# dnbaker/bonsai

Hardware: AMD Instinct MI355X
Metric: reads/s classified (150 bp) (higher is better)
Workload: dtype u64

## Files before the change

### bonsai_amd/context.py

```python
import ctypes as C
from fractions import Fraction

import numpy as np

from . import _lib
from ._lib import BonsaiAmdError, u8p, u16p, u32p, u64p, vp


def _p(a, t):
    return a.ctypes.data_as(t)


def concat_reads(seqs):
    bs = [s.encode() if isinstance(s, str) else bytes(s) for s in seqs]
    offsets = np.zeros(len(bs) + 1, dtype=np.uint64)
    if bs:
        offsets[1:] = np.cumsum([len(b) for b in bs], dtype=np.uint64)
    bases = np.frombuffer(b"".join(bs), dtype=np.uint8).copy() if bs else np.zeros(0, dtype=np.uint8)
    return bases, offsets


def pack_reads(bases, offsets, threads=1):
    L = _lib.load()
    bases = np.ascontiguousarray(bases, dtype=np.uint8)
# ... 32 lines not shown
                                        _p(offsets, u64p), _p(words, u64p), _p(bw, u64p), _p(bm, u32p), cap, C.cast(C.byref(nb), u64p), int(threads))
        if rc == 0:
            return words, bw[:nb.value].copy(), bm[:nb.value].copy(), offsets
        if nb.value <= cap:
            raise BonsaiAmdError("bns_pack_reads_qual_ptrs: %s" % L.bns_strerror(rc).decode())
        cap = int(nb.value)


def confidence_fraction(threshold):
    if isinstance(threshold, bool):
        raise ValueError("confidence threshold must be a number in [0, 1], not %r" % (threshold,))
    if isinstance(threshold, float):
        threshold = str(threshold)
    try:
        f = Fraction(threshold)
    except (TypeError, ValueError, ZeroDivisionError):
        raise ValueError("confidence threshold must be a number in [0, 1], not %r" % (threshold,)) from None
    if not 0 <= f <= 1:
        raise ValueError("confidence threshold must lie in [0, 1], not %s" % f)
    if f.denominator >= 1 << 64:
        raise ValueError("confidence threshold %s: num and den in lowest terms must be below 2^64" % f)
    return f.numerator, f.denominator


class Context:
    def __init__(self, device=0):
        self.L = _lib.load()
        h = vp()
        rc = self.L.bns_create(device, C.byref(h))
        if rc != 0:
            raise BonsaiAmdError("bns_create(%d): %s" % (device, self.L.bns_strerror(rc).decode()))
        self.h = h
        self.k = None

    def close(self):
        if getattr(self, "h", None):
            self.L.bns_destroy(self.h)
            self.h = None

    def __del__(self):
        try:
            self.close()
        except Exception:
            pass

    def _chk(self, rc, what):
        if rc != 0:
            raise BonsaiAmdError("%s: %s (%s)" % (what, self.L.bns_strerror(rc).decode(),
                                                   self.L.bns_last_error(self.h).decode()))

    def set_encoder(self, k, gaps=None, canonicalize=True, spaced_intended=True):
        g = None
        gp = None
        if gaps is not None:
            g = np.ascontiguousarray(gaps, dtype=np.uint16)
            if g.size != k - 1:
                raise ValueError("gaps must have k-1 entries")
            gp = _p(g, u16p)
        self._chk(self.L.bns_set_encoder(self.h, k, gp, int(canonicalize), int(spaced_intended)), "bns_set_encoder")
        self.k = k

    def set_window(self, w, score=_lib.SCORE_LEX):
        self._chk(self.L.bns_set_window(self.h, w, score), "bns_set_window")

    def set_bucket_slots_log2(self, lg):
        self._chk(self.L.bns_set_bucket_slots_log2(self.h, lg), "bns_set_bucket_slots_log2")

    def set_table_buckets(self, n):
        self._chk(self.L.bns_set_table_buckets(self.h, n), "bns_set_table_buckets")

    def set_minimizer_identity(self, bits):
        self._chk(self.L.bns_set_minimizer_identity(self.h, bits), "bns_set_minimizer_identity")

    def set_table_fill(self, mode):
        self._chk(self.L.bns_set_table_fill(self.h, mode), "bns_set_table_fill")

    def table_geometry(self):
        g = (C.c_uint64 * 8)()
        self._chk(self.L.bns_table_geometry(self.h, g), "bns_table_geometry")
        return {"buckets": g[0], "m": g[1], "identity_bits": g[2], "spilled_keys": g[3], "span": g[4], "overflow_keys": g[5], "group_fill": g[6]}

    def table_warning(self):
        return self.L.bns_table_warning(self.h).decode()

    def debug_set(self, bits):
        self._chk(self.L.bns_debug_set(self.h, bits), "bns_debug_set")

    def debug_claim_waves(self, waves):
        self._chk(self.L.bns_debug_set_claim_waves(self.h, int(waves)), "bns_debug_set_claim_waves")

    def last_classify_form(self):
        w = np.zeros(18, dtype=np.uint32)
        n = self.L.bns_debug_last_classify_form(self.h, _p(w, u32p), w.size)
        if n != w.size:
            raise BonsaiAmdError("bns_debug_last_classify_form: %d words" % n)
        v = [int(x) for x in w]
        return {"kernel": tuple(v[1:9]) if v[0] else None, "overflow_kernel": tuple(v[10:14]) if v[9] else None,
                "overflow_units": v[14], "overflow_grid": v[15], "chunk": v[16], "grid": v[17]}

    def load_table(self, n_buckets, flags, keys, vals, layout=_lib.LAYOUT_MINBUCKET):
        flags = np.ascontiguousarray(flags, dtype=np.uint32)
        keys = np.ascontiguousarray(keys, dtype=np.uint64)
        vals = np.ascontiguousarray(vals, dtype=np.uint32)
        if keys.size != n_buckets or vals.size != n_buckets or flags.size != max(1, n_buckets >> 4):
            raise ValueError("khash array sizes do not match n_buckets")
        self._chk(self.L.bns_load_table(self.h, n_buckets, _p(flags, u32p), _p(keys, u64p), _p(vals, u32p), layout),
                  "bns_load_table")

    def load_table_device(self, n_buckets, d_flags, d_keys, d_vals, layout=_lib.LAYOUT_MINBUCKET, stream=None):
        self._chk(self.L.bns_load_table_device(self.h, n_buckets, d_flags, d_keys, d_vals, layout, stream),
                  "bns_load_table_device")

    def table_info(self):
        nk = C.c_uint64(); nb = C.c_uint64(); ly = C.c_int()
        self._chk(self.L.bns_table_info(self.h, C.byref(nk), C.byref(nb), C.byref(ly)), "bns_table_info")
        return {"n_keys": nk.value, "device_bytes": nb.value, "layout": ly.value}

    def table_stats(self):
        st = (C.c_uint64 * 4)()
        self._chk(self.L.bns_table_stats(self.h, st), "bns_table_stats")
        return {"n_keys": st[0], "n_overflow_keys": st[1], "main_bytes": st[2], "overflow_bytes": st[3]}

    def set_minimizer_span(self, span):
        self._chk(self.L.bns_set_minimizer_span(self.h, span), "bns_set_minimizer_span")

    def table_minimizer(self):
        m = C.c_uint32(); sp = C.c_uint64()
        self._chk(self.L.bns_table_minimizer(self.h, C.byref(m), C.byref(sp)), "bns_table_minimizer")
        return {"m": m.value, "spilled_keys": sp.value}

    def load_taxonomy(self, parent):
        parent = np.ascontiguousarray(parent, dtype=np.uint32)
        self._chk(self.L.bns_load_taxonomy(self.h, _p(parent, u32p), parent.size), "bns_load_taxonomy")
        self._n_tax = int(parent.size)

    def tally_enable(self, on=True):
        self._chk(self.L.bns_tally_enable(self.h, int(bool(on))), "bns_tally_enable")

    def tally(self, reset=False):
        n = getattr(self, "_n_tax", 0)
        direct = np.zeros(n + 1, dtype=np.uint64)
        clade = np.zeros(n + 1, dtype=np.uint64)
        self._chk(self.L.bns_tally_read(self.h, _p(direct, u64p), _p(clade, u64p), n + 1, int(bool(reset))), "bns_tally_read")
        return direct, clade

    def table_tally(self):
        n = getattr(self, "_n_tax", 0)
        direct = np.zeros(n + 1, dtype=np.uint64)
        clade = np.zeros(n + 1, dtype=np.uint64)
        self._chk(self.L.bns_table_tally(self.h, _p(direct, u64p), _p(clade, u64p), n + 1), "bns_table_tally")
        return direct, clade

    def set_confidence(self, threshold):
        num, den = confidence_fraction(threshold)
        self._chk(self.L.bns_set_confidence(self.h, num, den), "bns_set_confidence")

    def set_min_hit_groups(self, n):
        self._chk(self.L.bns_set_min_hit_groups(self.h, int(n)), "bns_set_min_hit_groups")

    def sketch_enable(self, max_taxa=65536):
        self._chk(self.L.bns_sketch_enable(self.h, int(max_taxa)), "bns_sketch_enable")

    def sketch(self, reset=False):
        s = C.c_uint32(); dropped = C.c_uint32()
        self._chk(self.L.bns_sketch_read(self.h, None, None, 0, C.byref(s), C.byref(dropped), 0), "bns_sketch_read")
        bins = np.zeros(s.value, dtype=np.uint32)
# ... 399 lines not shown
```

### bonsai_amd/csrc/bns_api.hip

```cpp
#include "../../include/bonsai_amd.h"
#include "bns_kernels.hip"
#include "bns_tally.hpp"
#include "bns_inspect.hpp"
#include "bns_confidence.hpp"
#include "bns_sketch.hpp"
#include "bns_hit_groups.hpp"
#include "bns_text_plan.hpp"

#include <dlfcn.h>
#if defined(__x86_64__)
#include <immintrin.h>
#endif
#include <rccl/rccl.h>
#include <mutex>
#include <numeric>
#include <algorithm>
#include <array>
#include <cstdio>
#include <cstdlib>
#include <cmath>
#include <cstring>
#include <string>
#include <chrono>
#include <type_traits>
#include <thread>
#include <vector>

using namespace bns;

namespace {

struct DevBuf {
    void *p = nullptr;
    size_t cap = 0;
};

struct SmallLayout {
    u32 work_counter; u32 pad0[31];
    u32 ovf_count, max_len; u32 pad1[30];
    unsigned long long load_cnt[8];
    unsigned long long runs_cursor;
    unsigned long long lines_cursor;
};
constexpr size_t SMALL_BYTES = 512;
constexpr size_t SMALL_CLASSIFY_ZERO = offsetof(SmallLayout, max_len) + sizeof(u32);
static_assert(sizeof(SmallLayout) <= SMALL_BYTES, "ctx->small is allocated with SMALL_BYTES");
static_assert(offsetof(SmallLayout, load_cnt) >= SMALL_CLASSIFY_ZERO, "classify's memset must not reach the other entry points' words");

constexpr int BNS_DBG_PEXT_OFF = 0x400;
constexpr int BNS_DBG_FORCE_RCCL = 0x800;
constexpr int BNS_DBG_INSPECT_TINY = 0x8;
constexpr int BNS_DBG_INSPECT_WHOLE = 0x80;

struct ClassifyForm {
    enum { VALID, SPACED, LAYOUT, KT, NM, SPAN, OVC, WIDE, PACKED, OVF_LAUNCHED, OVF_SPACED, OVF_LAYOUT, OVF_WIDE, OVF_PACKED, OVF_UNITS,
           OVF_GRID, CHUNK, GRID, N_WORDS };
    u32 w[N_WORDS] = {0};
};

}

struct bns_text_work;
namespace bns { struct BuildSession; }
namespace bns { struct WindowSession; }
void text_work_free(struct bns_ctx *ctx);

struct bns_ctx {
    int device = 0;
    bns_text_work *text_work = nullptr;
    bns::BuildSession *build = nullptr;
    bns::WindowSession *windows = nullptr;
    hipStream_t stream = nullptr;
    hipStream_t copy_stream = nullptr;
    hipStream_t back_stream = nullptr;
    hipEvent_t slice_ev[16] = {}, done_ev[16] = {};
    std::string err;
    int n_cu = 256;
    bool enc_set = false;
    u32 k = 0, c = 0;
    bool canon = true, spaced = false, spaced_intended = false;
    u16 pos[32] = {0};
    u32 n_runs = 0;
    u8 run_start[32] = {0}, run_len[32] = {0};
    u64 sample_mask = 0;
    u32 table_m = 0;
    u32 min_span_req = 0;
    u64 n_spilled = 0;
    bool group_fill = false;
    u32 table_len = 0, table_shift = 0, table_canon = 1;
    u32 sp_run_len = 0, sp_run_shift = 0;
    u32 pext_on = 0, pext_n1 = 0, pext_steps[2] = {0, 0}, pext_top[2] = {0xFF, 0xFF};
    u64 pext_mask[2] = {0, 0}, pext_mv[2][6] = {{0}};
    u32 win = 0;
    int score = 0;
    int layout = -1;
    u64 kh_nb = 0;
    const u32 *kflags = nullptr;
    const u64 *kkeys = nullptr;
    const u32 *kvals = nullptr;
    bool own_khash = false;
    Slot *slots = nullptr;
    u64 n_slots = 0;
    u32 n_mb = 0;
    Slot *ovf_slots = nullptr;
    u64 n_ovf_slots = 0, n_ovf_keys = 0;
    u64 n_keys = 0;
    u32 slots_log2_req = 0;
    u64 n_buckets_req = 0;
    int fill_req = -1;
    int wide_req = -1;
    bool table_wide = false;
    u32 table_span = 0;
    std::string warn;
    int dbg = 0;
    unsigned claim_waves = 0;
    ClassifyForm last_form;
    u32 table_k = 0;
    TaxNode *nodes = nullptr;
    u32 n_nodes = 0;
    u32 tax_clock = 0;
    bool tally_on = false;
    DevBuf tally_direct, tally_clade, tally_scan;
    u64 conf_num = 0, conf_den = 1;
    DevBuf conf_hits;
    u32 min_hit_groups = 0;
    u32 sketch_cap = 0;
    DevBuf sk_regs, sk_slot_of, sk_slot_bin, sk_seen, sk_state;
// ... 50 lines not shown
{
    const u64 need = (items + per_block - 1) / per_block;
    const u64 cap = (u64)ctx->n_cu * blocks_per_cu;
    return (unsigned)std::max<u64>(1, std::min(need, cap));
}

template <class F>
void dispatch_sp_layout(bool spaced, int layout, F &&f)
{
    if (spaced) {
        if (layout == 2) f(std::true_type{}, std::integral_constant<int, 2>{});
        else if (layout == 1) f(std::true_type{}, std::integral_constant<int, 1>{});
        else f(std::true_type{}, std::integral_constant<int, 0>{});
    } else {
        if (layout == 2) f(std::false_type{}, std::integral_constant<int, 2>{});
        else if (layout == 1) f(std::false_type{}, std::integral_constant<int, 1>{});
        else f(std::false_type{}, std::integral_constant<int, 0>{});
    }
}

void free_table(bns_ctx *ctx)
{
    if (ctx->own_khash) {
        if (ctx->kflags) (void)hipFree((void *)ctx->kflags);
        if (ctx->kkeys) (void)hipFree((void *)ctx->kkeys);
        if (ctx->kvals) (void)hipFree((void *)ctx->kvals);
    }
    ctx->kflags = nullptr; ctx->kkeys = nullptr; ctx->kvals = nullptr; ctx->own_khash = false; ctx->kh_nb = 0;
    if (ctx->slots) (void)hipFree(ctx->slots);
    if (ctx->ovf_slots) (void)hipFree(ctx->ovf_slots);
    ctx->ovf_slots = nullptr; ctx->n_ovf_slots = 0; ctx->n_ovf_keys = 0;
    ctx->slots = nullptr; ctx->n_slots = 0; ctx->n_mb = 0; ctx->n_keys = 0; ctx->layout = -1; ctx->table_wide = false;
}

int ready(bns_ctx *ctx, bool need_table, bool need_tax)
{
    if (!ctx) return BNS_ERR_ARG;
    if (!ctx->enc_set) return fail(ctx, BNS_ERR_STATE, "encoder not configured (bns_set_encoder)");
    if (need_table && ctx->layout < 0) return fail(ctx, BNS_ERR_STATE, "no table loaded (bns_load_table)");
    if (need_table && ctx->layout == BNS_LAYOUT_MINBUCKET && ctx->table_k != ctx->k)
        return fail(ctx, BNS_ERR_STATE, "encoder k changed after a BNS_LAYOUT_MINBUCKET table was built; reload the table");
    if (need_tax && !ctx->nodes) return fail(ctx, BNS_ERR_STATE, "no taxonomy loaded (bns_load_taxonomy)");
    return BNS_OK;
}

}

#include "bns_classify.hpp"
#include "bns_dust.hpp"
#include "bns_build.hpp"
#include "bns_fewest.hpp"
#include "bns_minimize.hpp"
#include "bns_table_load.hpp"
#include "bns_windows.hpp"
#include "bns_hashers.hpp"

extern "C" {

int bns_version(void) { return 115; }

int bns_device_pci_bus_id(int device, char *out, int cap)
{
    if (!out || cap < 16) return BNS_ERR_ARG;
    return hipDeviceGetPCIBusId(out, cap, device) == hipSuccess ? BNS_OK : BNS_ERR_HIP;
}

int bns_device_count(void)
{
    int n = 0;
    if (hipGetDeviceCount(&n) != hipSuccess) return 0;
    return n;
}

int bns_debug_set(bns_ctx *ctx, int bits) { if (!ctx) return BNS_ERR_ARG; ctx->dbg = bits; return BNS_OK; }
int bns_debug_set_claim_waves(bns_ctx *ctx, unsigned waves) { if (!ctx || (waves & 3u)) return BNS_ERR_ARG; ctx->claim_waves = waves; return BNS_OK; }
int bns_debug_last_classify_form(const bns_ctx *ctx, uint32_t *out, int n)
{
    if (!ctx || !out || n < 0) return BNS_ERR_ARG;
    const int c = std::min<int>(n, ClassifyForm::N_WORDS);
    for (int i = 0; i < c; ++i) out[i] = ctx->last_form.w[i];
    return c;
}
#ifdef BNS_WAVE_TIMES
extern "C" int bns_debug_wave_times(bns_ctx *ctx, unsigned long long *out40960)
{
    if (!ctx || !out40960) return BNS_ERR_ARG;
    if (hipDeviceSynchronize() != hipSuccess) return BNS_ERR_HIP;
    if (hipMemcpyFromSymbol(out40960, HIP_SYMBOL(bns::g_wave_times), sizeof(bns::g_wave_times)) != hipSuccess) return BNS_ERR_HIP;
    return BNS_OK;
}
#endif
#ifdef BNS_COUNT_FETCHES
__global__ void ovf_stats_kernel(const bns::Slot *ovf, unsigned long long n_slots, unsigned long long *out)
{
    const unsigned long long stride = (unsigned long long)gridDim.x * blockDim.x;
    unsigned long long occ = 0, full = 0;
    for (unsigned long long b = (unsigned long long)blockIdx.x * blockDim.x + threadIdx.x; b < n_slots / 4; b += stride) {
        unsigned c = 0;
        for (int q = 0; q < 4; ++q) c += ovf[b * 4 + q].occ ? 1u : 0u;
        occ += c; full += c == 4u;
    }
    atomicAdd(out, occ); atomicAdd(out + 1, full);
}
extern "C" int bns_debug_ovf_stats(bns_ctx *ctx, unsigned long long *out3)
{
    if (!ctx || !out3) return BNS_ERR_ARG;
    out3[0] = out3[1] = 0; out3[2] = ctx->n_ovf_slots;
    if (!ctx->ovf_slots) return BNS_OK;
    unsigned long long *d = ((SmallLayout *)ctx->small.p)->load_cnt;
    if (hipMemset(d, 0, 16) != hipSuccess) return BNS_ERR_HIP;
    hipLaunchKernelGGL(ovf_stats_kernel, dim3(1024), dim3(256), 0, 0, ctx->ovf_slots, (unsigned long long)ctx->n_ovf_slots, d);
    if (hipDeviceSynchronize() != hipSuccess) return BNS_ERR_HIP;
    if (hipMemcpy(out3, d, 16, hipMemcpyDeviceToHost) != hipSuccess) return BNS_ERR_HIP;
    return BNS_OK;
}
extern "C" int bns_debug_ovf_copy(bns_ctx *ctx, void *host, unsigned long long bytes)
{
    if (!ctx || !host || !ctx->ovf_slots) return BNS_ERR_ARG;
    const unsigned long long have = ctx->n_ovf_slots * sizeof(bns::Slot);
    if (hipMemcpy(host, ctx->ovf_slots, bytes < have ? bytes : have, hipMemcpyDeviceToHost) != hipSuccess) return BNS_ERR_HIP;
    return BNS_OK;
}
extern "C" int bns_debug_fetch_count(bns_ctx *ctx, unsigned long long *out8)
{
    if (!ctx || !out8) return BNS_ERR_ARG;
    unsigned long long z[8] = {0, 0, 0, 0, 0, 0, 0, 0};
    if (hipDeviceSynchronize() != hipSuccess) return BNS_ERR_HIP;
    if (hipMemcpyFromSymbol(out8, HIP_SYMBOL(bns::g_fetch_count), sizeof(z)) != hipSuccess) return BNS_ERR_HIP;
    if (hipMemcpyToSymbol(HIP_SYMBOL(bns::g_fetch_count), z, sizeof(z)) != hipSuccess) return BNS_ERR_HIP;
    return BNS_OK;
}
#endif

const char *bns_strerror(int code)
{
    switch (code) {
        case BNS_OK: return "ok";
        case BNS_ERR_ARG: return "bad argument";
        case BNS_ERR_HIP: return "HIP runtime error";
        case BNS_ERR_NOMEM: return "out of memory";
        case BNS_ERR_STATE: return "context not ready";
        case BNS_ERR_TAX_CYCLE: return "taxonomy contains a cycle";
        case BNS_ERR_TAX_RANGE: return "taxid out of range for the flat parent array";
        case BNS_ERR_TABLE: return "inconsistent khash table";
        case BNS_ERR_NO_DEVICE: return "no usable GPU device";
        default: return "unknown error";
    }
}

const char *bns_last_error(const bns_ctx *ctx) { return ctx ? ctx->err.c_str() : "null context"; }

int bns_create(int device, bns_ctx **out)
{
    if (!out) return BNS_ERR_ARG;
    *out = nullptr;
    int n = 0;
    if (hipGetDeviceCount(&n) != hipSuccess || n <= 0 || device < 0 || device >= n) return BNS_ERR_NO_DEVICE;
    if (hipSetDevice(device) != hipSuccess) return BNS_ERR_NO_DEVICE;
    bns_ctx *ctx = new (std::nothrow) bns_ctx();
    if (!ctx) return BNS_ERR_NOMEM;
    ctx->device = device;
    hipDeviceProp_t prop;
    if (hipGetDeviceProperties(&prop, device) == hipSuccess) ctx->n_cu = prop.multiProcessorCount > 0 ? prop.multiProcessorCount : 256;
    if (hipStreamCreateWithFlags(&ctx->stream, hipStreamNonBlocking) != hipSuccess) { delete ctx; return BNS_ERR_HIP; }
    for (int i = 0; i < bns_ctx::EV_RING; ++i)
        if (hipEventCreate(&ctx->ev0[i]) != hipSuccess || hipEventCreate(&ctx->ev1[i]) != hipSuccess) { delete ctx; return BNS_ERR_HIP; }
    if (hipMalloc(&ctx->small.p, SMALL_BYTES) != hipSuccess) { delete ctx; return BNS_ERR_NOMEM; }
    ctx->small.cap = SMALL_BYTES;
    *out = ctx;
    return BNS_OK;
}
// ... 1026 lines not shown
```

### bonsai_amd/csrc/bns_claims.hpp

```cpp
#pragma once
#include <cstdint>

#if defined(__HIPCC__) || defined(__CUDACC__)
#define BNS_CLAIMS_HD __host__ __device__ __forceinline__
#else
#define BNS_CLAIMS_HD inline
#endif

namespace bns {


BNS_CLAIMS_HD uint32_t claim_stagger_prefix(uint32_t w, uint32_t full)
{
    const uint32_t q = w / full, r = w - q * full;
    return q * (full * (full + 1u) / 2u) + r * (r + 1u) / 2u;
}

BNS_CLAIMS_HD void claim_static(uint32_t w, uint32_t chunk, uint32_t full, uint32_t &base, uint32_t &size)
{
    if (chunk < full) { base = w * chunk; size = chunk; return; }
    base = claim_stagger_prefix(w, full);
    size = 1u + w % full;
}

BNS_CLAIMS_HD uint32_t claim_dynamic_base(uint32_t dyn_base, uint32_t d, uint32_t full) { return dyn_base + d * full; }

BNS_CLAIMS_HD uint32_t claim_cnt(uint32_t base, uint32_t size, uint32_t n_units)
{
    const uint32_t left = n_units - base;
    return left < size ? left : size;
}

inline void claim_geometry(uint64_t n_units, uint32_t max_blocks, uint32_t full, uint32_t &chunk, uint32_t &grid)
{
    const uint64_t W = (uint64_t)max_blocks * 4u;
    uint64_t share = (n_units + W - 1) / W;
    if (share < 4) share = 4;
    chunk = (uint32_t)(share < full ? share : full);
    const uint64_t need = ((n_units + chunk - 1) / chunk + 3) / 4;
    grid = (uint32_t)(need < max_blocks ? need : max_blocks);
    if (grid < 1) grid = 1;
}

inline uint32_t claim_dynamic_start(uint64_t n_units, uint32_t launched, uint32_t chunk, uint32_t full)
{
    if (chunk < full) return (uint32_t)n_units;
    const uint64_t stat = claim_stagger_prefix(launched, full);
    return (uint32_t)(stat < n_units ? stat : n_units);
}

}
```

### bonsai_amd/csrc/bns_classify.hpp

```cpp
#pragma once
#include <utility>

namespace {

int tally_units(bns_ctx *ctx, const u32 *d_taxon, u64 n_units, hipStream_t st, bool neg);
int sketch_units(bns_ctx *ctx, const ClassifyParams &p, hipStream_t st);
int hit_groups_units(bns_ctx *ctx, const ClassifyParams &p, hipStream_t st);
int dust_image_span(bns_ctx *ctx, const u64 *words, const u32 *nmask, const u64 *offsets, u64 n_seqs, u64 lo, u64 hi, hipStream_t st);

void fill_params(const bns_ctx *ctx, ClassifyParams &p)
{
    std::memset(&p, 0, sizeof(p));
    p.words = (const u64 *)ctx->words.p;
    p.nmask = (const u32 *)ctx->nmask.p;
    p.slots = ctx->layout == BNS_LAYOUT_MINBUCKET ? ctx->ovf_slots : ctx->slots;
    p.ovf_mask = ctx->n_ovf_slots ? ctx->n_ovf_slots / 4 - 1 : 0;
    p.minb = reinterpret_cast<const MinBucket *>(ctx->slots);
    p.bucket_mask = (ctx->n_slots && ctx->layout == BNS_LAYOUT_BUCKET) ? ctx->n_slots / 4 - 1 : 0;
    p.n_mb = ctx->layout == BNS_LAYOUT_MINBUCKET ? ctx->n_mb : 0u;
    p.min_wide = ctx->table_wide ? 1u : 0u;
    p.kflags = ctx->kflags; p.kkeys = ctx->kkeys; p.kvals = ctx->kvals; p.kh_nb = ctx->kh_nb;
    p.nodes = ctx->nodes; p.n_nodes = ctx->n_nodes;
    p.k = ctx->k; p.c = ctx->c; p.canon = ctx->canon ? 1 : 0; p.dbg = ctx->dbg;
    std::memcpy(p.pos, ctx->pos, sizeof(p.pos));
// ... 59 lines not shown
    hipLaunchKernelGGL((classify_overflow_kernel<SP, LY, WIDE, PACKED>), dim3(grid), dim3(64), 0, st, p, scratch, total_bases);
}

template <class Forms, class Key, class F, size_t... I>
bool with_form(const Forms &forms, const Key &key, F &&f, std::index_sequence<I...>)
{
    return ((forms[I] == key ? (f(std::integral_constant<size_t, I>{}), true) : false) || ...);
}

int launch_form(bns_ctx *ctx, const ClassifyFormKey &key, const ClassifyParams &p, unsigned grid, hipStream_t st)
{
    const bool found = with_form(CLASSIFY_FORMS, key, [&](auto i) {
        constexpr ClassifyFormKey K = CLASSIFY_FORMS[decltype(i)::value];
        unsigned g = grid;
        if constexpr (K.kt == 0 && !K.wide) {
            int per_cu = 8;
            if (hipOccupancyMaxActiveBlocksPerMultiprocessor(&per_cu, classify_kernel<K.spaced, K.layout, K.kt, K.nm, K.span, K.ovc, K.wide, K.packed>, 256, 0) != hipSuccess || per_cu < 1) per_cu = 8;
            g = std::min<unsigned>(grid, (unsigned)ctx->n_cu * (unsigned)std::min(per_cu, 8));
        }
        launch_classify<K.spaced, K.layout, K.kt, K.nm, K.span, K.ovc, K.wide, K.packed>(ctx->last_form, p, g, st);
    }, std::make_index_sequence<CLASSIFY_FORMS.size()>{});
    return found ? BNS_OK : fail(ctx, BNS_ERR_STATE, "classify: the form chosen for this call is not among the compiled ones");
}
int launch_overflow_form(bns_ctx *ctx, const OverflowFormKey &key, const ClassifyParams &p, u32 n_units, unsigned grid, hipStream_t st, u32 *scratch,
                         u64 total_bases)
{
    const bool found = with_form(OVERFLOW_FORMS, key, [&](auto i) {
        constexpr OverflowFormKey K = OVERFLOW_FORMS[decltype(i)::value];
        launch_classify_overflow<K.spaced, K.layout, K.wide, K.packed>(ctx->last_form, p, n_units, grid, st, scratch, total_bases);
    }, std::make_index_sequence<OVERFLOW_FORMS.size()>{});
    return found ? BNS_OK : fail(ctx, BNS_ERR_STATE, "classify: the overflow form chosen for this call is not among the compiled ones");
}


struct ClassifyIn {
    const char *bases = nullptr; const u64 *words = nullptr; const u32 *nmask = nullptr;
    const u64 *offsets = nullptr; u64 n_reads = 0, total_bases = 0; u32 max_read_len = 0; int paired = 0;
    bool masked = false;
    u64 first_base = 0, end_base = 0;
};
struct UnitOut { u32 *taxon = nullptr, *missing = nullptr, *ambig = nullptr, *n_hits = nullptr, *hits = nullptr; };

struct ClassifyLaunch {
    hipStream_t st = nullptr; int nm = 1; u64 n_units = 0; bool packed = false, can_overflow = false;
    ClassifyParams p;
};

int classify_check(bns_ctx *ctx, const ClassifyIn &in, const UnitOut &out)
{
    BNS_RC(ready(ctx, true, true));
    if (!in.offsets || !out.taxon || (!in.bases && !in.words && in.total_bases)) return BNS_ERR_ARG;
    if (in.paired && (in.n_reads & 1)) return fail(ctx, BNS_ERR_ARG, "paired input needs an even number of reads");
    return BNS_OK;
}

int classify_prepare(bns_ctx *ctx, const ClassifyIn &in, const UnitOut &out, ClassifyLaunch &L)
{
    hipStream_t st = L.st;
    SmallLayout *sm = (SmallLayout *)ctx->small.p;
    HIPCHK(ctx, hipMemsetAsync(sm, 0, SMALL_CLASSIFY_ZERO, st));
    u32 max_read_len = in.max_read_len;
    if (max_read_len == 0) {
        hipLaunchKernelGGL(max_len_kernel, dim3(grid_for(ctx, in.n_reads, 256)), dim3(256), 0, st, in.offsets, (u64)in.n_reads, &sm->max_len);
        HIPCHK(ctx, hipGetLastError());
        HIPCHK(ctx, hipMemcpyAsync(&max_read_len, &sm->max_len, 4, hipMemcpyDeviceToHost, st));
        HIPCHK(ctx, hipStreamSynchronize(st));
    }
    L.can_overflow = unit_can_overflow(L.nm, max_read_len, ctx->c);
    if (L.can_overflow) BNS_RC(ensure(ctx, ctx->ovf_list, (size_t)L.n_units * 8));

    ClassifyParams &p = L.p;
    fill_params(ctx, p);
    p.offsets = in.offsets; p.n_units = L.n_units; p.nmates = L.nm; p.bases = (const u8 *)in.bases;
    if (L.packed) { p.words = in.words; p.nmask = in.nmask; }
    p.taxon = out.taxon; p.missing = out.missing; p.ambig = out.ambig; p.n_hits = out.n_hits; p.hits = out.hits;
    if ((ctx->conf_num || ctx->sketch_cap) && !out.hits) {
        BNS_RC(ensure(ctx, ctx->conf_hits, (size_t)in.total_bases * 4 + 4));
        p.hits = (u32 *)ctx->conf_hits.p;
    }
    p.want_hits = p.hits ? 1 : 0;
    BNS_RC(ensure(ctx, ctx->records, (size_t)L.n_units * 16));
    p.records = (uint4 *)ctx->records.p;
    p.ovf_count = &sm->ovf_count; p.ovf_list = L.can_overflow ? (u64 *)ctx->ovf_list.p : nullptr;
    p.work_counter = &sm->work_counter;
    p.emit_none = (ctx->spaced && !ctx->spaced_intended) ? 1 : 0;
    return BNS_OK;
}

int classify_launch(bns_ctx *ctx, const ClassifyLaunch &L)
{
    hipStream_t st = L.st;
    unsigned grid = (unsigned)ctx->n_cu * 8u;
    if (ctx->claim_waves) grid = std::max(1u, std::min(grid, ctx->claim_waves / 4u));
    const int evi = ctx->ev_head;
    if (ctx->timing) HIPCHK(ctx, hipEventRecord(ctx->ev0[evi], st));
    const bool heavy = ovf_heavy(ctx->dbg, ctx->n_ovf_keys, ctx->n_keys);
    BNS_RC(launch_form(ctx, choose_form(L.p.k, L.p.m, ctx->canon, ctx->spaced, ctx->layout, ctx->table_wide, heavy, L.packed, L.nm), L.p, grid, st));
    HIPCHK(ctx, hipGetLastError());
    if (ctx->timing) {
        HIPCHK(ctx, hipEventRecord(ctx->ev1[evi], st));
        ctx->ev_head = (evi + 1) % bns_ctx::EV_RING;
        ctx->ev_count = std::min(ctx->ev_count + 1, (int)bns_ctx::EV_RING);
    }
    return BNS_OK;
}

int classify_overflow_pass(bns_ctx *ctx, const ClassifyIn &in, const ClassifyLaunch &L)
{
    hipStream_t st = L.st;
    u32 h_ovf = 0;
    HIPCHK(ctx, hipMemcpyAsync(&h_ovf, L.p.ovf_count, 4, hipMemcpyDeviceToHost, st));
    HIPCHK(ctx, hipStreamSynchronize(st));
    if (!h_ovf) return BNS_OK;
    BNS_RC(ensure(ctx, ctx->scratch, (size_t)in.total_bases * 16));
    const unsigned grid = std::min<u32>(h_ovf, (u32)ctx->n_cu * 8);
    BNS_RC(launch_overflow_form(ctx, choose_overflow_form(ctx->spaced, ctx->layout, ctx->table_wide, L.packed), L.p, h_ovf, grid, st, (u32 *)ctx->scratch.p,
                                (u64)in.total_bases));
    HIPCHK(ctx, hipGetLastError());
    return BNS_OK;
}

int classify_finish(bns_ctx *ctx, const ClassifyIn &in, const UnitOut &out, const ClassifyLaunch &L)
{
    hipStream_t st = L.st;
    const u64 n_units = L.n_units;
    const bool hit_groups = ctx->min_hit_groups >= 2;
    ClassifyParams p = L.p;
    if ((hit_groups || ctx->sketch_cap) && in.bases) {
        BNS_RC(pack_reads(ctx, in.bases, in.offsets, in.n_reads, in.total_bases, st));
        p.words = (const u64 *)ctx->words.p; p.nmask = (const u32 *)ctx->nmask.p;
    }
    if (ctx->conf_num) {
        hipLaunchKernelGGL(confidence_kernel, dim3(grid_for(ctx, (n_units + CONF_GROUP - 1) / CONF_GROUP, 4)), dim3(256), 0, st, (uint4 *)ctx->records.p,
                           (const u64 *)in.offsets, (u32)L.nm, (const u32 *)L.p.hits, (u64)n_units, (const TaxNode *)ctx->nodes, ctx->n_nodes, ctx->conf_num,
                           ctx->conf_den);
        HIPCHK(ctx, hipGetLastError());
    }
    if (hit_groups) BNS_RC(hit_groups_units(ctx, p, st));
    hipLaunchKernelGGL(unpack_kernel, dim3(grid_for(ctx, n_units, 256)), dim3(256), 0, st, (const uint4 *)ctx->records.p, (u64)n_units,
                       out.taxon, out.missing, out.ambig, out.n_hits);
    HIPCHK(ctx, hipGetLastError());
    BNS_RC(tally_units(ctx, out.taxon, n_units, st, false));
    if (!ctx->sketch_cap) return BNS_OK;
    return sketch_units(ctx, p, st);
}

int classify_device_impl(bns_ctx *ctx, const ClassifyIn &in0, const UnitOut &out, void *stream)
{
    BNS_RC(classify_check(ctx, in0, out));
    HIPCHK(ctx, hipSetDevice(ctx->device));
    ClassifyIn in = in0;
    ClassifyLaunch L;
    L.st = stream ? (hipStream_t)stream : ctx->stream;
    L.nm = in.paired ? 2 : 1;
    L.n_units = in.n_reads / (u64)L.nm;
    if (L.n_units == 0) return BNS_OK;
    if (too_many_units(L.n_units)) return fail(ctx, BNS_ERR_ARG, "more than 2^32 - 2^22 units in one batch: split it");
    if (ctx->dust_w && !in.masked && (in.bases || in.words)) {
        const u64 lo = in.end_base ? in.first_base : 0, hi = in.end_base ? in.end_base : in.total_bases;
        if (in.bases) {
            BNS_RC(pack_reads(ctx, in.bases, in.offsets, in.n_reads, in.total_bases, L.st));
            BNS_RC(dust_image_span(ctx, (const u64 *)ctx->words.p, (const u32 *)ctx->nmask.p, in.offsets, in.n_reads, lo, hi, L.st));
        } else BNS_RC(dust_image_span(ctx, in.words, in.nmask, in.offsets, in.n_reads, lo, hi, L.st));
        in.bases = nullptr; in.words = (const u64 *)ctx->words.p; in.nmask = (const u32 *)ctx->nmask.p;
    }
    L.packed = in.words != nullptr;
    BNS_RC(classify_prepare(ctx, in, out, L));
// ... 305 lines not shown
```

### bonsai_amd/csrc/bns_classify_plan.hpp

```cpp
#pragma once
#include <array>
#include <cstddef>
#include "bns_table_plan.hpp"

namespace bns {

constexpr int BNS_DBG_OVC_OFF = 0x2000;
constexpr int BNS_DBG_OVC_ON = 0x8000;

constexpr u32 LDS_CAP = 128;

struct ClassifyFormKey {
    bool spaced; int layout, kt, nm, span; bool ovc, wide, packed;
    constexpr bool operator==(const ClassifyFormKey &o) const
    {
        return spaced == o.spaced && layout == o.layout && kt == o.kt && nm == o.nm && span == o.span && ovc == o.ovc && wide == o.wide && packed == o.packed;
    }
};
struct OverflowFormKey {
    bool spaced; int layout; bool wide, packed;
    constexpr bool operator==(const OverflowFormKey &o) const { return spaced == o.spaced && layout == o.layout && wide == o.wide && packed == o.packed; }
};

constexpr u32 FIXED_K_FULL = 31;
constexpr u32 FIXED_K_USUAL[4] = {21, 25, 27, 32};
constexpr int GENERIC_SPAN = 8;

constexpr bool fixed_k_window(u32 k, u32 m)
{
    bool common = k == FIXED_K_FULL;
    for (u32 ku : FIXED_K_USUAL) common = common || k == ku;
    if (!common) return false;
    for (const MinCand &c : MIN_CANDS) if (minimizer_len(k, c) == m) return true;
    return false;
}

constexpr ClassifyFormKey choose_form(u32 k, u32 m, bool canon, bool spaced, int layout, bool table_wide, bool heavy, bool packed, int nmates)
{
    const int ly = layout == BNS_LAYOUT_MINBUCKET ? 2 : (layout == BNS_LAYOUT_BUCKET ? 1 : 0);
    const bool clustered = !spaced && ly == 2;
    const bool wide = clustered && table_wide;
    if (clustered && canon && fixed_k_window(k, m)) {
        const int nm = nmates == 1 ? 1 : 2;
        if (!(heavy || wide || packed)) return {false, 2, (int)k, nm, (int)(k - m), false, false, false};
        if (k == FIXED_K_FULL && !(packed && (heavy || wide))) return {false, 2, (int)k, nm, (int)(k - m), heavy, wide, packed};
    }
    return {spaced, ly, 0, 0, GENERIC_SPAN, false, wide, packed};
}

constexpr OverflowFormKey choose_overflow_form(bool spaced, int layout, bool table_wide, bool packed)
{
    const int ly = layout == BNS_LAYOUT_MINBUCKET ? 2 : (layout == BNS_LAYOUT_BUCKET ? 1 : 0);
    return {spaced, ly, !spaced && ly == 2 && table_wide, packed};
}

constexpr bool ovf_heavy(int dbg, u64 n_ovf_keys, u64 n_keys)
{
    return (dbg & BNS_DBG_OVC_ON) || (!(dbg & BNS_DBG_OVC_OFF) && n_ovf_keys * 1000ULL > n_keys);
}

constexpr u64 max_unit_kmers(int nmates, u32 max_read_len, u32 c) { return max_read_len >= c ? (u64)nmates * (max_read_len - c + 1) : 0; }
constexpr bool unit_can_overflow(int nmates, u32 max_read_len, u32 c) { return max_unit_kmers(nmates, max_read_len, c) > LDS_CAP; }

constexpr u64 MAX_CLASSIFY_UNITS = (1ULL << 32) - (1ULL << 22);
constexpr bool too_many_units(u64 n_units) { return n_units >= MAX_CLASSIFY_UNITS; }

constexpr size_t win_scratch_bytes(bool spaced, bool canon, int score, u32 win, u32 c, unsigned grid)
{
    const bool stream_windows = !spaced && (!canon || score == BNS_SCORE_ENTROPY_STRING);
    if (!stream_windows || win <= c || win - c + 1 <= 64) return 0;
    return (size_t)grid * 4 * ((size_t)2 * (win - c + 65u) * 8);
}

template <class K, size_t CAP>
struct FormSet {
    K v[CAP] = {};
    size_t n = 0;
    constexpr bool has(const K &key) const { for (size_t i = 0; i < n; ++i) if (v[i] == key) return true; return false; }
    constexpr void add(const K &key) { if (!has(key)) v[n++] = key; }
};
struct FormSets { FormSet<ClassifyFormKey, 96> kern; FormSet<OverflowFormKey, 24> ovf; };

constexpr FormSets enumerate_forms()
{
    FormSets s;
    for (u32 k = 1; k <= 32; ++k)
        for (int spaced = 0; spaced < 2; ++spaced)
            for (int layout = 0; layout < 3; ++layout) {
                if (spaced && k < 2) continue;
                const bool clustered = !spaced && layout == 2;
                for (u32 ci = 0; ci < (clustered ? 3u : 1u); ++ci)
// ... 26 lines not shown
```

### bonsai_amd/csrc/bns_kernels.hip

```cpp
#include "bns_device.hpp"
#include "bns_kernels.hpp"

namespace bns {

typedef const volatile __attribute__((address_space(4))) ClassifyParams ColdParams;
__device__ __forceinline__ ColdParams *cold_params() { return (ColdParams *)__builtin_amdgcn_kernarg_segment_ptr(); }

__device__ __forceinline__ u32 base_code(u32 b, u32 &bad)
{
    const u32 c = b & 0xDFu;
    const bool ok = (c == 0x41u) | (c == 0x43u) | (c == 0x47u) | (c == 0x54u);
    const u32 x = (c >> 1) & 3u;
    bad = ok ? 0u : 1u;
    return ok ? (x ^ (x >> 1)) : 0u;
}

__global__ __launch_bounds__(256) void pack_kernel(const u8 *__restrict__ bases, const u64 *__restrict__ offsets,
                                                   u64 n_reads, u64 *__restrict__ words, u32 *__restrict__ nmask)
{
    const int lane = lane_id();
    const u64 wave = (u64)blockIdx.x * (blockDim.x >> 6) + (u64)__builtin_amdgcn_readfirstlane((int)(threadIdx.x >> 6));
    const u64 n_waves = (u64)gridDim.x * (blockDim.x >> 6);
    for (u64 r = wave; r < n_reads; r += n_waves) {
        const u64 o = offsets[r];
// ... 991 lines not shown
                        }
                    }
                }
            } else {
                for (u32 rd = 0; rd * 64u < chunk_nk; ++rd) {
                    const u32 jl = rd * 64u + (u32)lane;
                    u64 kmer, win = 0;
                    bool valid;
                    if (SPACED) valid = p.n_runs ? extract_spaced_lds(pk, rd, p, rdesc, kmer, clean) : extract_spaced(W, M, rd, k, rdesc, kmer);
                    else        { extract_lds32(pk, rd, k, clean, win, valid); kmer = win >> (64u - 2u * k); }
                    valid = valid && jl < chunk_nk;
                    pad_valu<BNS_PAD_VALU>(lane);
                    pad_vfast<BNS_PAD_VFAST>(lane);
                    pad_salu<BNS_PAD_SALU>();
                    pad_lds<BNS_PAD_LDS>(lane);
                    const u64 kf = kmer;
                    const u64 krc = SPACED ? 0ULL : revcomp_top(win, k);
                    if (!SPACED && (KT != 0 || p.canon)) kmer = kf < krc ? kf : krc;
                    ProbeResult pr;
#ifdef BNS_ABLATION
                    if (p.dbg & 1) { pr.found = valid && (kmer & 1); pr.val = 1000u + (u32)(kmer & 3); }
                    else
#endif
                    if (LAYOUT == 2) {
                        u32 minh;
                        if (SPACED) minh = key_minhash(kmer, k, MinSpec{p.m, p.min_len, p.min_shift, p.min_canon, 0u});
                        else if (WIDE) minh = wide_bucket_in(round_minhash_wide<MW>(kf, krc, rd, k, mlen, reinterpret_cast<u64 *>(ring)), mlen);
                        else minh = round_minhash<MW, (KT != 0 && SPAN == 15)>(kf, krc, rd, k, mlen, ring);
#ifdef BNS_ABLATION
                        if (p.dbg & 4) minh = (u32)wang64(kmer);
#endif
                        pr = probe_minbucket<(KT == 0 || KT == 32), NB, OVC, true, OVC>(p.minb, kmer, bucket_of(minh, n_mb), valid, aux, p.slots, p.ovf_mask,
                                                                                         OVC ? minb_tagbit(minh) : 0u);
                    } else if (LAYOUT == 1) pr = probe_bucket(p.slots, p.bucket_mask, kmer, valid);
                    else                  pr = probe_khash(p.kflags, p.kkeys, p.kvals, p.kh_nb, kmer, valid);
                    const u64 fm = tally(pr, valid);
#ifdef BNS_ABLATION
                    u64 rem = (p.dbg & 2) ? 0ULL : fm;
#else
                    u64 rem = fm;
#endif
                    while (rem) {
                        const int l = __builtin_ctzll(rem);
                        const u32 t = readlane(pr.val, l);
                        const u64 mm = ballot64(pr.val == t) & fm;
                        rem &= ~mm;
                        const u32 c = (u32)__popcll(mm);
                        const bool eq = ckey == t;
                        if (ballot64(eq) & dmask) { ccnt = eq ? ccnt + c : ccnt; continue; }
                        if (!counter_insert(ckey, ccnt, dmask, keys, cnt, cap, D, t, c)) { overflow = true; break; }
                    }
                }
            }
        }
        if (m == 0) ambig = L - c + 1u - n_hits - missing;
        else        ambig += L - (c - 1u) - n_hits - missing;
    }

    ColdParams *kp = cold_params();
    if (overflow && record_overflow) {
        if (lane == 0) {
            u32 *oc = kp->ovf_count;
            u64 *ol = kp->ovf_list;
            if (ol) { const u32 slot = atomicAdd(oc, 1u); ol[slot] = u; }
        }
        rec_valid = false;
        return;
    }
    u32 taxon;
    if (D <= 1u) taxon = D ? readlane(ckey, 0) : 0u;
    else if (D <= 64u) taxon = resolve_regs(ckey, ccnt, D, kp->nodes, kp->n_nodes);
    else {
        u32 l2 = (u32)lane;
        asm volatile("" : "+v"(l2));
        keys[l2] = ckey; cnt[l2] = ccnt;
        __builtin_amdgcn_wave_barrier();
        taxon = resolve_wave(keys, cnt, tin, tout, D, kp->nodes, kp->n_nodes, (int)(l2 & 63u));
    }
    rec_out = make_uint4(taxon, missing, ambig, n_hits);
    rec_valid = true;
}

#ifdef BNS_WAVE_TIMES
constexpr int WAVE_STAMPS = 5;
__device__ unsigned long long g_wave_times[WAVE_STAMPS * 8192];
#endif
template <bool SPACED, int LAYOUT, int KT, int NM, int SPAN = 8, bool OVC = false, bool WIDE = false, bool PACKED = false>
__global__ __launch_bounds__(256, (ClassifyTraits<SPACED, LAYOUT, KT, NM, SPAN, OVC, WIDE, PACKED>::WAVES)) void classify_kernel(ClassifyParams p)
{
    using T = ClassifyTraits<SPACED, LAYOUT, KT, NM, SPAN, OVC, WIDE, PACKED>;
    __shared__ __attribute__((aligned(8))) u32 s_ring[4][T::RING_U32];
    __shared__ __attribute__((aligned(16))) u32 s_mh[4][T::AUX_U32];
    __shared__ u64 s_pk[4][IMG_U64];
    const int wv = __builtin_amdgcn_readfirstlane((int)(threadIdx.x >> 6));
    u32 *ctr_keys, *ctr_cnt;
    if constexpr (T::PAIRS) {
        ctr_keys = s_mh[wv] + minb_aux_u32(16); ctr_cnt = ctr_keys + LDS_CAP;
    } else {
        __shared__ u32 s_keys[4][LDS_CAP], s_cnt[4][LDS_CAP];
        ctr_keys = s_keys[wv]; ctr_cnt = s_cnt[wv];
    }
    const int lane = lane_id();
#ifdef BNS_WAVE_TIMES
    struct TimeStamp {
        unsigned long long t[WAVE_STAMPS]; u32 slot;
        __device__ ~TimeStamp() { if ((threadIdx.x & 63u) == 0 && slot < 8192u) { t[4] = wall_clock64(); for (int i = 0; i < WAVE_STAMPS; ++i) g_wave_times[WAVE_STAMPS * slot + i] = t[i]; } }
    } stamp{{(unsigned long long)wall_clock64(), 0, 0, 0, 0}, blockIdx.x * 4u + (u32)wv};
#endif
    const u32 n_units = (u32)p.n_units;
    const u32 nm = NM ? (u32)NM : (u32)p.nmates;
    const u32 FULL = classify_chunk(nm);
    auto claim = [&]() -> u32 { u32 *const c = cold_params()->work_counter; return c && lane == 0 ? atomicAdd(c, 1u) : 0u; };
    auto load_offs = [&](u32 base, u32 cnt) -> u64 {
        const u64 *op = const_cast<const u64 *>(cold_params()->offsets) + (u64)base * nm;
        return (u32)lane <= cnt * nm ? op[lane] : 0ULL;
    };
    u32 base, cnt;
    claim_static(blockIdx.x * 4u + (u32)wv, p.chunk, FULL, base, cnt);
#ifdef BNS_WAVE_TIMES
    stamp.t[1] = wall_clock64();
#endif
    if (base >= n_units) return;
    cnt = claim_cnt(base, cnt, n_units);
    u64 offs = load_offs(base, cnt);
    Prefetch pre;
    {
        const u64 o0 = readlane64(offs, 0);
        prefetch_clear<PACKED>(pre);
        prefetch_issue<PACKED>(p, (u64)base * nm, o0, readlane((u32)offs, 1) - (u32)o0, pre);
    }
    uint4 pend = make_uint4(0, 0, 0, 0);
    u32 pend_u = 0;
    bool pend_valid = false;
    for (;;) {
        u32 next_v = 0;
        u32 nbase = 0xFFFFFFFFu;
        u64 noffs = 0;
        const u32 jload = cnt > 2u ? cnt - 2u : 0u;
        for (u32 j = 0; j < cnt; ++j) {
            if (j == jload) {
                if (j == 0u) next_v = claim();
                nbase = claim_dynamic_base(cold_params()->claim_base, (u32)__builtin_amdgcn_readfirstlane((int)next_v), FULL);
                if (nbase < n_units) noffs = load_offs(nbase, claim_cnt(nbase, FULL, n_units));
            }
            Prefetch npre;
            auto issue_next = [&]() __attribute__((always_inline)) {
                prefetch_clear<PACKED>(npre);
                u64 n0 = 0, nr = 0;
                u32 nL = 0;
                if (j + 1u < cnt) {
                    n0 = readlane64(offs, (int)((j + 1u) * nm));
                    nL = readlane((u32)offs, (int)((j + 1u) * nm + 1u)) - (u32)n0;
                    nr = (u64)(base + j + 1u) * nm;
                } else if (nbase < n_units) {
                    n0 = readlane64(noffs, 0);
                    nL = readlane((u32)noffs, 1) - (u32)n0;
                    nr = (u64)nbase * nm;
                }
                prefetch_issue<PACKED>(p, nr, n0, nL, npre);
                if (j + 1u == jload) next_v = claim();
                if (pend_valid && lane == 0) cold_params()->records[pend_u] = pend;
            };
            classify_unit<SPACED, LAYOUT, KT, NM, SPAN, OVC, WIDE, PACKED>(p, base + j, offs, j * nm, true, pre, ctr_keys, ctr_cnt, s_mh[wv] + MINB_LIST_U32,
                                          s_mh[wv] + MINB_LIST_U32 + LDS_CAP, LDS_CAP, true, s_ring[wv], s_mh[wv], s_pk[wv], pend, pend_valid, issue_next);
            pend_u = base + j;
            pre = npre;
#ifdef BNS_WAVE_TIMES
            stamp.t[3] = wall_clock64();
            if (!stamp.t[2]) stamp.t[2] = stamp.t[3];
#endif
        }
        if (nbase >= n_units) break;
        base = nbase; offs = noffs;
        cnt = claim_cnt(base, FULL, n_units);
    }
    if (pend_valid && lane == 0) cold_params()->records[pend_u] = pend;
}

template <bool SPACED, int LAYOUT, bool WIDE = false, bool PACKED = false>
__global__ __launch_bounds__(64) void classify_overflow_kernel(ClassifyParams p, u32 *scratch, u64 total_bases)
{
    using T = ClassifyTraits<SPACED, LAYOUT, 0, 0, 8, false, WIDE, PACKED, true>;
    __shared__ __attribute__((aligned(8))) u32 s_ring[T::RING_U32];
    __shared__ __attribute__((aligned(16))) u32 s_mh[T::AUX_U32];
    __shared__ u64 s_pk[IMG_U64];
    const u32 n = *p.ovf_count;
    for (u32 i = blockIdx.x; i < n; i += gridDim.x) {
        const u64 u = p.ovf_list[i];
        const u64 b0 = p.offsets[u * (u64)p.nmates];
        const u64 bm = p.offsets[u * (u64)p.nmates + 1];
        const u64 b1 = p.offsets[(u + 1) * (u64)p.nmates];
        uint4 rec;
        bool ok;
        const u64 offv = (threadIdx.x & 63u) == 0 ? b0 : ((threadIdx.x & 63u) == 1 ? bm : b1);
        classify_unit<SPACED, LAYOUT, 0, 0, 8, false, WIDE, PACKED, true>(p, u, offv, 0u, false, Prefetch{0u, 0u, 0u}, scratch + b0, scratch + total_bases + b0,
                                      scratch + 2 * total_bases + b0, scratch + 3 * total_bases + b0, (u32)(b1 - b0), false, s_ring, s_mh, s_pk, rec, ok, [] {});
        if (ok && threadIdx.x == 0) p.records[u] = rec;
    }
}

template <bool SPACED>
__global__ __launch_bounds__(256) void encode_kernel(ClassifyParams p, u64 *__restrict__ kmers, u32 *__restrict__ n_kmers)
{
    __shared__ u64 s_win[4][256];
    const int lane = lane_id();
    const u32 rdesc = SPACED ? run_desc(p) : 0u;
    const u64 wave = (u64)blockIdx.x * 4 + (u64)__builtin_amdgcn_readfirstlane((int)(threadIdx.x >> 6));
    const u64 n_waves = (u64)gridDim.x * 4;
    const u32 k = p.k, c = p.c;
    const bool windowed = p.w > c;
    const u32 span = windowed ? p.w : c;
    const u32 rounds_per_chunk = (2048u - (span - 1u)) / 64u;
    u64 *win = s_win[__builtin_amdgcn_readfirstlane((int)(threadIdx.x >> 6))];
    if (!SPACED && windowed && (!p.canon || p.score == 2)) {
        for (u64 r = wave; r < p.n_units; r += n_waves) {
            const u64 o = p.offsets[r];
            u32 emitted = 0;
            auto put = [&](u64 kmer, bool on) {
                const u64 vm = ballot64(on);
                if (on) kmers[o + emitted + (u32)__popcll(vm & lanemask_lt())] = kmer;
                emitted += (u32)__popcll(vm);
            };
            if (p.w - p.k + 1u > 64u) uncanon_windowed_seq<true>(p, r, p.win_scratch + wave * 2 * (u64)(p.w - p.k + 65u), put);
            else                      uncanon_windowed_seq<false>(p, r, win, put);
            if (lane == 0) n_kmers[r] = emitted;
        }
        return;
    }
    for (u64 r = wave; r < p.n_units; r += n_waves) {
        const u64 o = p.offsets[r];
        const u32 L = (u32)(p.offsets[r + 1] - o);
        const u64 wb = (o >> 5) + r;
        const u32 n_words = (L + 31u) >> 5;
        const u32 nk = (L >= span && !p.emit_none) ? L - span + 1u : 0u;
        u32 emitted = 0;
        for (u32 j0 = 0; j0 < nk; j0 += rounds_per_chunk * 64u) {
            const u32 wi = (j0 >> 5) + (u32)lane;
            const u64 W = wi < n_words ? p.words[wb + wi] : 0ULL;
            const u32 M = wi < n_words ? p.nmask[wb + wi] : 0xFFFFFFFFu;
            const u32 chunk_nk = (nk - j0) < rounds_per_chunk * 64u ? (nk - j0) : rounds_per_chunk * 64u;
            for (u32 rd = 0; rd * 64u < chunk_nk; ++rd) {
                const u32 jl = rd * 64u + (u32)lane;
                u64 kmer;
                bool valid;
                if (windowed) { kmer = windowed_round<SPACED>(W, M, rd, p, rdesc, win); valid = !SPACED || kmer != ~0ULL; }
                else if (SPACED) valid = p.n_runs ? extract_spaced_runs(W, M, rd, p, rdesc, kmer) : extract_spaced(W, M, rd, k, rdesc, kmer);
                else        valid = extract_unspaced(W, M, rd, k, kmer);
                valid = valid && jl < chunk_nk;
                if (!SPACED && !windowed && p.canon) kmer = canonical(kmer, k);
                const u64 vm = ballot64(valid);
                if (valid) kmers[o + emitted + (u32)__popcll(vm & lanemask_lt())] = kmer;
                emitted += (u32)__popcll(vm);
            }
        }
        if (lane == 0) n_kmers[r] = emitted;
    }
// ... 497 lines not shown
```

Measured before the change: 2.186 billion.

## Shard dynamic work-claim counter per XCC with cross-shard stealing

Replaces the single global atomic work counter with eight padded counters, one per XCC (read from the hardware XCC_ID register), and interleaves chunk indices across the shards. When a wave's home shard runs dry, it moves on to the other shards' counters to steal the remaining work. The aim is to cut cross-die atomic contention and latency on the claim path of the MI355X's multiple XCCs. The cost is extra loop structure, a restarted prefetch pipeline after each steal, and some imbalance near the tail.

```diff
diff --git a/bonsai_amd/context.py b/bonsai_amd/context.py
--- a/bonsai_amd/context.py
+++ b/bonsai_amd/context.py
@@ -138,6 +138,8 @@
 
     def table_warning(self):
         return self.L.bns_table_warning(self.h).decode()
+
+    DBG_SHARD_BY_WAVE = 0x200000
 
     def debug_set(self, bits):
         self._chk(self.L.bns_debug_set(self.h, bits), "bns_debug_set")
diff --git a/bonsai_amd/csrc/bns_api.hip b/bonsai_amd/csrc/bns_api.hip
--- a/bonsai_amd/csrc/bns_api.hip
+++ b/bonsai_amd/csrc/bns_api.hip
@@ -36,13 +36,13 @@
 };
 
 struct SmallLayout {
-    u32 work_counter; u32 pad0[31];
+    u32 work_counter[CLAIM_SHARDS][CLAIM_COUNTER_STRIDE];
     u32 ovf_count, max_len; u32 pad1[30];
     unsigned long long load_cnt[8];
     unsigned long long runs_cursor;
     unsigned long long lines_cursor;
 };
-constexpr size_t SMALL_BYTES = 512;
+constexpr size_t SMALL_BYTES = 1536;
 constexpr size_t SMALL_CLASSIFY_ZERO = offsetof(SmallLayout, max_len) + sizeof(u32);
 static_assert(sizeof(SmallLayout) <= SMALL_BYTES, "ctx->small is allocated with SMALL_BYTES");
 static_assert(offsetof(SmallLayout, load_cnt) >= SMALL_CLASSIFY_ZERO, "classify's memset must not reach the other entry points' words");
@@ -259,11 +259,11 @@
     return c;
 }
 #ifdef BNS_WAVE_TIMES
-extern "C" int bns_debug_wave_times(bns_ctx *ctx, unsigned long long *out40960)
-{
-    if (!ctx || !out40960) return BNS_ERR_ARG;
+extern "C" int bns_debug_wave_times(bns_ctx *ctx, unsigned long long *out65536)
+{
+    if (!ctx || !out65536) return BNS_ERR_ARG;
     if (hipDeviceSynchronize() != hipSuccess) return BNS_ERR_HIP;
-    if (hipMemcpyFromSymbol(out40960, HIP_SYMBOL(bns::g_wave_times), sizeof(bns::g_wave_times)) != hipSuccess) return BNS_ERR_HIP;
+    if (hipMemcpyFromSymbol(out65536, HIP_SYMBOL(bns::g_wave_times), sizeof(bns::g_wave_times)) != hipSuccess) return BNS_ERR_HIP;
     return BNS_OK;
 }
 #endif
diff --git a/bonsai_amd/csrc/bns_claims.hpp b/bonsai_amd/csrc/bns_claims.hpp
--- a/bonsai_amd/csrc/bns_claims.hpp
+++ b/bonsai_amd/csrc/bns_claims.hpp
@@ -22,6 +22,10 @@
     base = claim_stagger_prefix(w, full);
     size = 1u + w % full;
 }
+
+constexpr uint32_t CLAIM_SHARDS = 8;
+constexpr uint32_t CLAIM_COUNTER_STRIDE = 32;
+BNS_CLAIMS_HD uint32_t claim_shard_global(uint32_t d, uint32_t x) { return d * CLAIM_SHARDS + x; }
 
 BNS_CLAIMS_HD uint32_t claim_dynamic_base(uint32_t dyn_base, uint32_t d, uint32_t full) { return dyn_base + d * full; }
 
diff --git a/bonsai_amd/csrc/bns_classify.hpp b/bonsai_amd/csrc/bns_classify.hpp
--- a/bonsai_amd/csrc/bns_classify.hpp
+++ b/bonsai_amd/csrc/bns_classify.hpp
@@ -165,7 +165,7 @@
     BNS_RC(ensure(ctx, ctx->records, (size_t)L.n_units * 16));
     p.records = (uint4 *)ctx->records.p;
     p.ovf_count = &sm->ovf_count; p.ovf_list = L.can_overflow ? (u64 *)ctx->ovf_list.p : nullptr;
-    p.work_counter = &sm->work_counter;
+    p.work_counter = &sm->work_counter[0][0];
     p.emit_none = (ctx->spaced && !ctx->spaced_intended) ? 1 : 0;
     return BNS_OK;
 }
diff --git a/bonsai_amd/csrc/bns_classify_plan.hpp b/bonsai_amd/csrc/bns_classify_plan.hpp
--- a/bonsai_amd/csrc/bns_classify_plan.hpp
+++ b/bonsai_amd/csrc/bns_classify_plan.hpp
@@ -7,6 +7,7 @@
 
 constexpr int BNS_DBG_OVC_OFF = 0x2000;
 constexpr int BNS_DBG_OVC_ON = 0x8000;
+constexpr int BNS_DBG_SHARD_BY_WAVE = 0x200000;
 
 constexpr u32 LDS_CAP = 128;
 
diff --git a/bonsai_amd/csrc/bns_kernels.hip b/bonsai_amd/csrc/bns_kernels.hip
--- a/bonsai_amd/csrc/bns_kernels.hip
+++ b/bonsai_amd/csrc/bns_kernels.hip
@@ -1097,7 +1097,7 @@
 }
 
 #ifdef BNS_WAVE_TIMES
-constexpr int WAVE_STAMPS = 5;
+constexpr int WAVE_STAMPS = 8;
 __device__ unsigned long long g_wave_times[WAVE_STAMPS * 8192];
 #endif
 template <bool SPACED, int LAYOUT, int KT, int NM, int SPAN = 8, bool OVC = false, bool WIDE = false, bool PACKED = false>
@@ -1120,12 +1120,35 @@
     struct TimeStamp {
         unsigned long long t[WAVE_STAMPS]; u32 slot;
         __device__ ~TimeStamp() { if ((threadIdx.x & 63u) == 0 && slot < 8192u) { t[4] = wall_clock64(); for (int i = 0; i < WAVE_STAMPS; ++i) g_wave_times[WAVE_STAMPS * slot + i] = t[i]; } }
-    } stamp{{(unsigned long long)wall_clock64(), 0, 0, 0, 0}, blockIdx.x * 4u + (u32)wv};
+    } stamp{{(unsigned long long)wall_clock64(), 0, 0, 0, 0, 0, 0, 0}, blockIdx.x * 4u + (u32)wv};
 #endif
     const u32 n_units = (u32)p.n_units;
     const u32 nm = NM ? (u32)NM : (u32)p.nmates;
     const u32 FULL = classify_chunk(nm);
-    auto claim = [&]() -> u32 { u32 *const c = cold_params()->work_counter; return c && lane == 0 ? atomicAdd(c, 1u) : 0u; };
+    auto home_shard = [&]() -> u32 {
+        u32 x;
+        asm("s_getreg_b32 %0, hwreg(HW_REG_XCC_ID, 0, 3)" : "=s"(x));
+        if (cold_params()->dbg & BNS_DBG_SHARD_BY_WAVE) x = blockIdx.x * 4u + (u32)wv;
+        return x & (CLAIM_SHARDS - 1u);
+    };
+    u32 shard = home_shard();
+    auto claim = [&]() -> u32 {
+        u32 *const c = cold_params()->work_counter;
+        return c && lane == 0 ? atomicAdd(c + shard * CLAIM_COUNTER_STRIDE, 1u) : 0u;
+    };
+    auto look = [&](u32 v) -> u32 {
+#ifdef BNS_WAVE_TIMES
+        const unsigned long long t0 = wall_clock64();
+        u32 d;
+        asm volatile("v_readfirstlane_b32 %0, %1" : "=s"(d) : "v"(v));
+        const unsigned long long dt = wall_clock64() - t0;
+        stamp.t[5] += dt; stamp.t[6] += 1u;
+        if (dt > stamp.t[7]) stamp.t[7] = dt;
+        return d;
+#else
+        return (u32)__builtin_amdgcn_readfirstlane((int)v);
+#endif
+    };
     auto load_offs = [&](u32 base, u32 cnt) -> u64 {
         const u64 *op = const_cast<const u64 *>(cold_params()->offsets) + (u64)base * nm;
         return (u32)lane <= cnt * nm ? op[lane] : 0ULL;
@@ -1137,56 +1160,68 @@
 #endif
     if (base >= n_units) return;
     cnt = claim_cnt(base, cnt, n_units);
-    u64 offs = load_offs(base, cnt);
-    Prefetch pre;
-    {
-        const u64 o0 = readlane64(offs, 0);
-        prefetch_clear<PACKED>(pre);
-        prefetch_issue<PACKED>(p, (u64)base * nm, o0, readlane((u32)offs, 1) - (u32)o0, pre);
-    }
     uint4 pend = make_uint4(0, 0, 0, 0);
     u32 pend_u = 0;
     bool pend_valid = false;
     for (;;) {
-        u32 next_v = 0;
-        u32 nbase = 0xFFFFFFFFu;
-        u64 noffs = 0;
-        const u32 jload = cnt > 2u ? cnt - 2u : 0u;
-        for (u32 j = 0; j < cnt; ++j) {
-            if (j == jload) {
-                if (j == 0u) next_v = claim();
-                nbase = claim_dynamic_base(cold_params()->claim_base, (u32)__builtin_amdgcn_readfirstlane((int)next_v), FULL);
-                if (nbase < n_units) noffs = load_offs(nbase, claim_cnt(nbase, FULL, n_units));
-            }
-            Prefetch npre;
-            auto issue_next = [&]() __attribute__((always_inline)) {
-                prefetch_clear<PACKED>(npre);
-                u64 n0 = 0, nr = 0;
-                u32 nL = 0;
-                if (j + 1u < cnt) {
-                    n0 = readlane64(offs, (int)((j + 1u) * nm));
-                    nL = readlane((u32)offs, (int)((j + 1u) * nm + 1u)) - (u32)n0;
-                    nr = (u64)(base + j + 1u) * nm;
-                } else if (nbase < n_units) {
-                    n0 = readlane64(noffs, 0);
-                    nL = readlane((u32)noffs, 1) - (u32)n0;
-                    nr = (u64)nbase * nm;
+        u64 offs = load_offs(base, cnt);
+        Prefetch pre;
+        {
+            const u64 o0 = readlane64(offs, 0);
+            prefetch_clear<PACKED>(pre);
+            prefetch_issue<PACKED>(p, (u64)base * nm, o0, readlane((u32)offs, 1) - (u32)o0, pre);
+        }
+        u32 nbase;
+        for (;;) {
+            u32 next_v = 0;
+            nbase = 0xFFFFFFFFu;
+            u64 noffs = 0;
+            const u32 jload = cnt > 2u ? cnt - 2u : 0u;
+            for (u32 j = 0; j < cnt; ++j) {
+                if (j == jload) {
+                    if (j == 0u) next_v = claim();
+                    nbase = claim_dynamic_base(cold_params()->claim_base, claim_shard_global(look(next_v), shard), FULL);
+                    if (nbase < n_units) noffs = load_offs(nbase, claim_cnt(nbase, FULL, n_units));
                 }
-                prefetch_issue<PACKED>(p, nr, n0, nL, npre);
-                if (j + 1u == jload) next_v = claim();
-                if (pend_valid && lane == 0) cold_params()->records[pend_u] = pend;
-            };
-            classify_unit<SPACED, LAYOUT, KT, NM, SPAN, OVC, WIDE, PACKED>(p, base + j, offs, j * nm, true, pre, ctr_keys, ctr_cnt, s_mh[wv] + MINB_LIST_U32,
-                                          s_mh[wv] + MINB_LIST_U32 + LDS_CAP, LDS_CAP, true, s_ring[wv], s_mh[wv], s_pk[wv], pend, pend_valid, issue_next);
-            pend_u = base + j;
-            pre = npre;
+                Prefetch npre;
+                auto issue_next = [&]() __attribute__((always_inline)) {
+                    prefetch_clear<PACKED>(npre);
+                    u64 n0 = 0, nr = 0;
+                    u32 nL = 0;
+                    if (j + 1u < cnt) {
+                        n0 = readlane64(offs, (int)((j + 1u) * nm));
+                        nL = readlane((u32)offs, (int)((j + 1u) * nm + 1u)) - (u32)n0;
+                        nr = (u64)(base + j + 1u) * nm;
+                    } else if (nbase < n_units) {
+                        n0 = readlane64(noffs, 0);
+                        nL = readlane((u32)noffs, 1) - (u32)n0;
+                        nr = (u64)nbase * nm;
+                    }
+                    prefetch_issue<PACKED>(p, nr, n0, nL, npre);
+                    if (j + 1u == jload) next_v = claim();
+                    if (pend_valid && lane == 0) cold_params()->records[pend_u] = pend;
+                };
+                classify_unit<SPACED, LAYOUT, KT, NM, SPAN, OVC, WIDE, PACKED>(p, base + j, offs, j * nm, true, pre, ctr_keys, ctr_cnt, s_mh[wv] + MINB_LIST_U32,
+                                              s_mh[wv] + MINB_LIST_U32 + LDS_CAP, LDS_CAP, true, s_ring[wv], s_mh[wv], s_pk[wv], pend, pend_valid, issue_next);
+                pend_u = base + j;
+                pre = npre;
 #ifdef BNS_WAVE_TIMES
-            stamp.t[3] = wall_clock64();
-            if (!stamp.t[2]) stamp.t[2] = stamp.t[3];
+                stamp.t[3] = wall_clock64();
+                if (!stamp.t[2]) stamp.t[2] = stamp.t[3];
 #endif
+            }
+            if (nbase >= n_units) break;
+            base = nbase; offs = noffs;
+            cnt = claim_cnt(base, FULL, n_units);
+        }
+        if (!cold_params()->work_counter) break;
+        const u32 home = home_shard();
+        while ((shard = (shard + 1u) & (CLAIM_SHARDS - 1u)) != home) {
+            nbase = claim_dynamic_base(cold_params()->claim_base, claim_shard_global(look(claim()), shard), FULL);
+            if (nbase < n_units) break;
         }
         if (nbase >= n_units) break;
-        base = nbase; offs = noffs;
+        base = nbase;
         cnt = claim_cnt(base, FULL, n_units);
     }
     if (pend_valid && lane == 0) cold_params()->records[pend_u] = pend;
```

Measured after the change: 2.273 billion (median of 6 runs). 3.9% higher.
